# marcin-ochman/modular-slam

Hardware: AMD Instinct MI355X
Metric: ORB keypoints extracted+matched /sec, 640×480 RGB-D, 1/2/4/8 GPU; HBM GB/s vs roofline (higher is better)
Workload: dtype u8

## Files before the change

### modular-slam_amd/__init__.py

```python
import ctypes as C
import os
import subprocess

import numpy as np

_HERE = os.path.dirname(os.path.abspath(__file__))
LIB_PATH = os.path.join(_HERE, "libmslam_hip.so")

OK, E_INVALID, E_RUNTIME, E_CAPACITY, E_NO_VOCABULARY, E_FORMAT, E_NO_MODEL = range(7)
DBG_PYRAMID, DBG_BLURRED, DBG_CANDIDATES, DBG_SELECTED, DBG_CELLS, DBG_FORMS, DBG_QUAD_DIRECT = range(7)
QUAD_DIRECT_MAX_CANDIDATES = 1024
MATCHER_AUTO, MATCHER_POPCOUNT = 0, 1
DETECTOR_DISTRIBUTED, DETECTOR_CV_ORB = 0, 1
BOW_ASSIGN_TREE, BOW_ASSIGN_FLAT = 0, 1
CV_ORDER_LIBSTDCXX, CV_ORDER_RASTER = 0, 1
POSE_GRAPH_MAX_KEYFRAMES, POSE_GRAPH_MAX_EDGES = 1024, 65536

ABI_SYMBOLS = [
    "mslam_hip_default_params", "mslam_hip_abi_version", "mslam_hip_create", "mslam_hip_destroy",
    "mslam_hip_last_error", "mslam_hip_sync", "mslam_hip_detect", "mslam_hip_detect_batch_dev",
    "mslam_hip_get_batch_view", "mslam_hip_match", "mslam_hip_match_knn2", "mslam_hip_match_batch_dev",
    "mslam_hip_bow_load", "mslam_hip_bow_info", "mslam_hip_bow_words", "mslam_hip_bow_transform",
    "mslam_hip_bow_score", "mslam_hip_bow_db_add", "mslam_hip_bow_db_query", "mslam_hip_bow_db_clear",
    "mslam_hip_bow_batch_dev", "mslam_hip_get_bow_view", "mslam_hip_bow_cross_score_dev", "mslam_hip_level_geometry", "mslam_hip_debug_read",
    "mslam_hip_set_profiling", "mslam_hip_get_stage_times", "mslam_hip_copy_to_host", "mslam_hip_backproject", "mslam_hip_backproject_batch_dev",
    "mslam_hip_get_points_view", "mslam_hip_set_matcher", "mslam_hip_get_matcher",
    "mslam_hip_bow_pack_dev", "mslam_hip_bow_cross_score_packed_dev", "mslam_hip_debug_counts",
    "mslam_hip_last_match_kernel",
    "mslam_hip_join_matcher", "mslam_hip_bow_db_remove", "mslam_hip_bow_set_assignment",
    "mslam_hip_bow_db_reserve", "mslam_hip_bow_db_size", "mslam_hip_qlz_decompress",
    "mslam_hip_pnp_ransac", "mslam_hip_pnp_batch_dev", "mslam_hip_get_pnp_view", "mslam_hip_pnp_set_confidence", "mslam_hip_pack_batch_dev", "mslam_hip_packed_capacity",
    "mslam_hip_set_cv_keypoint_order", "mslam_hip_pnp_min_mse", "mslam_hip_pnp_min_mse_batch_dev",
    "mslam_hip_kf_add", "mslam_hip_kf_add_from_batch_dev", "mslam_hip_kf_remove", "mslam_hip_kf_clear", "mslam_hip_kf_size",
    "mslam_hip_kf_reserve", "mslam_hip_kf_read", "mslam_hip_relocalize",
    "mslam_hip_kf_visible", "mslam_hip_track", "mslam_hip_track_window", "mslam_hip_track_window_dev",
    "mslam_hip_kf_add_ids", "mslam_hip_kf_read_ids", "mslam_hip_kf_covisible", "mslam_hip_kf_union", "mslam_hip_kf_union_dev",
    "mslam_hip_match_guided_knn2", "mslam_hip_match_guided", "mslam_hip_set_guided_match", "mslam_hip_get_guided_match",
    "mslam_hip_bundle_adjust", "mslam_hip_bundle_adjust_global", "mslam_hip_kf_update_world", "mslam_hip_pose_graph",
]


class MslamHipError(RuntimeError):
    def __init__(self, code, msg):
        super().__init__("mslam_hip error %d: %s" % (code, msg))
        self.code = code


class Params(C.Structure):
    _fields_ = [("width", C.c_int32), ("height", C.c_int32), ("max_batch", C.c_int32), ("n_levels", C.c_int32),
                ("scale_factor", C.c_float), ("ini_fast_thr", C.c_int32), ("min_fast_thr", C.c_int32),
                ("min_node_area", C.c_uint32), ("max_keypoints", C.c_int32), ("max_candidates", C.c_int32),
                ("device", C.c_int32), ("stream", C.c_void_p), ("detector", C.c_int32), ("n_features", C.c_int32),
                ("edge_threshold", C.c_int32)]


class BatchView(C.Structure):
    _fields_ = [("n_frames", C.c_int32), ("capacity", C.c_int32), ("xy", C.c_void_p), ("desc", C.c_void_p),
                ("octave", C.c_void_p), ("angle", C.c_void_p), ("response", C.c_void_p), ("count", C.c_void_p),
                ("match_from", C.c_void_p), ("match_to", C.c_void_p), ("match_count", C.c_void_p)]


class PointsView(C.Structure):
    _fields_ = [("capacity", C.c_int32), ("xyz", C.c_void_p), ("valid", C.c_void_p)]

# ... 1298 lines not shown
```

### modular-slam_amd/csrc/api.hip

```cpp
#include "context.hpp"

#include <cfloat>
#include <climits>
#include <cmath>
#include <cstdio>
#include <cstring>
#include <cstdlib>
#include <algorithm>

using namespace mslam;

static thread_local std::string g_create_error;

#define ENTER(c)                                                                                                       \
    do                                                                                                                 \
    {                                                                                                                  \
        if(!(c))                                                                                                       \
            return MSLAM_HIP_E_INVALID;                                                                                \
        MSLAM_CHK(c, hipSetDevice((c)->p.device));                                                                     \
    } while(0)

static inline int cv_round_f(float v) { return (int)lrintf(v); }
static inline int cv_floor_f(float v)
{
// ... 616 lines not shown
        {
            const char* e = getenv("MSLAM_HIP_FUSED_LEVELS");
            const int want = e ? atoi(e) : kMaxLevels;
            const char* k = getenv("MSLAM_HIP_LEVEL_K6");
            const char* ks = getenv("MSLAM_HIP_LEVEL_K6_SMALL");
            c->level_k6_small = ks ? std::max(0, atoi(ks)) : 0;
            {
                const char* lc = getenv("MSLAM_HIP_LEVEL_CHAIN");
                const char* lf = getenv("MSLAM_HIP_LEVEL_CHAIN_FRAMES");
                const char* lw = getenv("MSLAM_HIP_LEVEL_CHAIN_WAVES");
                const char* lk = getenv("MSLAM_HIP_LEVEL_CHAIN_K6");
                c->level_chain = lc ? atoi(lc) : 0;
                c->level_chain_frames = lf ? std::max(1, std::min(64, atoi(lf))) : 2;
                c->level_chain_waves = lw ? atoi(lw) : 8;
                if(c->level_chain_waves != 4)
                    c->level_chain_waves = 8;
                c->level_chain_k6 = lk ? std::max(1, std::min(9, atoi(lk))) : 9;
            }
            c->level_k6 = k ? std::max(1, atoi(k)) : 5;
            const bool fits = (p.width & 3) == 0 && (double)B * p.width * p.height * 3 < 4294967296.0 &&
                              (double)B * g.slab < 4294901760.0  && (size_t)B * (p.width / 4) < (1u << 22) && p.height >= 8;
            int n_fused = fits ? 1 : 0;
            while(n_fused >= 1 && n_fused < p.n_levels && c->rs_q[n_fused] != SIZE_MAX && g.lv[n_fused].h >= 8 &&
                  (size_t)B * ((g.lv[n_fused].w + 3) / 4) < (1u << 22))
                ++n_fused;
            c->fused_levels = std::max(0, std::min(want, n_fused));
            const char* t = getenv("MSLAM_HIP_TILED_BLUR");
            c->geom.blur_tiled = c->fused_levels == p.n_levels && !(t && atoi(t) == 0) ? 1 : 0;
        }
        std::vector<BlurWave> bw;
        build_blur_waves(g, c->fused_levels, bw);
        c->blur_wpf = (int)bw.size();
        if(!bw.empty())
        {
            MSLAM_CHK(c, c->d_blur_waves.alloc(bw.size()));
            MSLAM_CHK(c, hipMemcpy(c->d_blur_waves, bw.data(), bw.size() * sizeof(BlurWave), hipMemcpyHostToDevice));
        }
    }
    MSLAM_CHK(c, c->d_cell_cnt.alloc(B * g.n_cells));
    MSLAM_CHK(c, c->d_cell_kp.alloc(B * g.n_cells * (size_t)kCellCap));
    QuadArgs& q = c->quad;
    MSLAM_CHK(c, c->q_cand.alloc(B * L * cap));
    MSLAM_CHK(c, c->q_cand_cnt.alloc(B * L));
    MSLAM_CHK(c, c->q_sel.alloc(B * L * cap));
    MSLAM_CHK(c, c->q_sel_cnt.alloc(B * L));
    MSLAM_CHK(c, c->q_kp_node.alloc(B * L * cap));
    MSLAM_CHK(c, c->q_nodes_a.alloc(B * L * cap));
    MSLAM_CHK(c, c->q_nodes_b.alloc(B * L * cap));
    MSLAM_CHK(c, c->q_ncnt_a.alloc(B * L * cap));
    MSLAM_CHK(c, c->q_ncnt_b.alloc(B * L * cap));
    MSLAM_CHK(c, c->q_child_cnt.alloc(B * L * cap * 4));
    MSLAM_CHK(c, c->q_ninfo.alloc(B * L * cap));
    MSLAM_CHK(c, c->q_best.alloc(B * L * cap));
    q.cand = c->q_cand, q.cand_cnt = c->q_cand_cnt, q.sel = c->q_sel, q.sel_cnt = c->q_sel_cnt, q.kp_node = c->q_kp_node;
    q.nodes_a = c->q_nodes_a, q.nodes_b = c->q_nodes_b, q.ncnt_a = c->q_ncnt_a, q.ncnt_b = c->q_ncnt_b;
    q.child_cnt = c->q_child_cnt, q.ninfo = c->q_ninfo, q.best = c->q_best;
    q.cell_cnt = c->d_cell_cnt;
    q.cell_kp = c->d_cell_kp;
    q.flags = c->d_flags;
    q.cand_cap = p.max_candidates;
    q.min_size = p.min_node_area;
    }

    for(auto& o : c->out)
    {
        MSLAM_CHK(c, o.xy.alloc((B + 1) * K * 2));
        MSLAM_CHK(c, o.desc.alloc((B + 1) * K * 32));
        MSLAM_CHK(c, o.octave.alloc((B + 1) * K));
        MSLAM_CHK(c, o.angle.alloc((B + 1) * K));
        MSLAM_CHK(c, o.response.alloc((B + 1) * K));
        MSLAM_CHK(c, o.count.alloc(B + 1));
        MSLAM_CHK(c, hipMemset(o.count, 0, (B + 1) * 4));
        MSLAM_CHK(c, o.idx0.alloc(B * K));
        MSLAM_CHK(c, o.idx1.alloc(B * K));
        MSLAM_CHK(c, o.dist0.alloc(B * K));
        MSLAM_CHK(c, o.dist1.alloc(B * K));
        MSLAM_CHK(c, o.mfrom.alloc(B * K));
        MSLAM_CHK(c, o.mto.alloc(B * K));
        MSLAM_CHK(c, o.mcount.alloc(B));
        MSLAM_CHK(c, hipMemset(o.mcount, 0, B * 4));
        MSLAM_CHK(c, hipEventCreateWithFlags(&o.ev_detect, hipEventDisableTiming));
        MSLAM_CHK(c, hipEventCreateWithFlags(&o.ev_match, hipEventDisableTiming));
    }
    MSLAM_CHK(c, hipStreamCreateWithFlags(&c->stream_m, hipStreamNonBlocking));
    {
        const char* e = getenv("MSLAM_HIP_OVERLAP_MATCH");
        c->overlap_match = !(e && atoi(e) == 0);
        auto on = [](const char* name) { const char* v = getenv(name); return !v || atoi(v) != 0; };
        c->knob_mirror_results = on("MSLAM_HIP_MIRROR_RESULTS");
        c->knob_zero_copy = on("MSLAM_HIP_ZERO_COPY_FRAME");
        c->knob_match_graph = on("MSLAM_HIP_MATCH_GRAPH");
        const char* zm = getenv("MSLAM_HIP_ZERO_COPY_MAX_BYTES");
        c->zero_copy_max_bytes = zm ? (size_t)atoll(zm) : (size_t)1200000;
        const char* m = getenv("MSLAM_HIP_MATCHER");
        c->matcher_kind = (m && std::strcmp(m, "popcount") == 0) ? MSLAM_HIP_MATCHER_POPCOUNT : MSLAM_HIP_MATCHER_AUTO;
    }
    c->cur = 0;
    MSLAM_CHK(c, hipDeviceSynchronize());
    return MSLAM_HIP_OK;
}

int mslam_hip_create(const mslam_hip_params* p, mslam_hip_ctx** out)
{
    if(!p || !out)
    {
        g_create_error = "null argument";
        return MSLAM_HIP_E_INVALID;
    }
    *out = nullptr;
// ... 1050 lines not shown
```

### modular-slam_amd/csrc/common.hpp

```cpp
#pragma once
#include <hip/hip_runtime.h>
#include <cstdint>
#include <cstddef>

namespace mslam
{

constexpr int kMaxLevels = 16;
constexpr int kBorder = 19;
constexpr int kCell = 64;
constexpr int kOverlap = 6;
constexpr int kCellCap = 1024;

constexpr size_t al256(size_t x) { return (x + 255) & ~(size_t)255; }

struct LevelGeom
{
    int w, h;
    int pitch;
    int offset;
    float scale;
    int bw, bh;
    int cell_base;
    int n_cells;
// ... 48 lines not shown
__host__ __device__ inline int kp_y(uint32_t p) { return (int)(p >> 20); }
__host__ __device__ inline int kp_score(uint32_t p) { return (int)(p & 0xFFu); }

enum : uint32_t
{
    kFlagCandOverflow = 1u,
    kFlagKpOverflow = 2u,
    kFlagQuadNoConverge = 4u,
    kFlagBowPackOverflow = 8u,
    kFlagDbFull = 16u,
    kFlagPackOverflow = 32u,
    kFlagUnionOverflow = 64u
};

void launch_gray(const uint8_t* d_bgr, uint8_t* d_pyr, const Geometry& g, int frame0, int n_frames, hipStream_t s);
void launch_resize(uint8_t* d_pyr, const Geometry& g, int level, const int32_t* d_xofs, const uint32_t* d_xcoef,
                   const int32_t* d_yofs, const uint32_t* d_ycoef, int frame0, int n_frames, hipStream_t s);
struct ResizeColArgs
{
    uint8_t* pyr;
    unsigned slab;
    int src_off, sh, spitch, dst_off, dw, dh, dpitch;
    const uint4* qt;
    const int32_t* yofs;
    const uint32_t* ycoef;
    int frame0, n_frames;
    int quads;
    float inv_quads;
    int R;
    int need_mask;
    int exact;
};
void launch_resize_col(const ResizeColArgs& a, hipStream_t s);
void launch_fast(const uint8_t* d_pyr, const Geometry& g, const CellDesc* d_cells, uint32_t* d_cell_cnt,
                 uint32_t* d_cell_kp, int ini_thr, int min_thr, int frame0, int n_frames, hipStream_t s);
void launch_denorm_selfcheck(uint32_t* d_out, hipStream_t s);
struct QuadArgs
{
    const uint32_t* cell_cnt;
    const uint32_t* cell_kp;
    uint32_t* cand;
    uint32_t* cand_cnt;
    uint32_t* sel;
    uint32_t* sel_cnt;
    uint32_t* kp_node;
    uint2* nodes_a;
    uint2* nodes_b;
    uint32_t* ncnt_a;
    uint32_t* ncnt_b;
    uint32_t* child_cnt;
    uint32_t* ninfo;
    uint32_t* best;
    uint32_t* flags;
    int cand_cap;
    unsigned min_size;
};
void launch_quadtree(const Geometry& g, const QuadArgs& a, int frame0, int n_frames, hipStream_t s);
int quad_depth_bound(const LevelGeom& lv, unsigned min_size);
unsigned quad_direct_levels(const Geometry& g);
struct BlurK
{
    uint32_t ta[3], tb[4], tc[4];
    uint32_t t01, t23, t45, t6;
};
BlurK make_blur_k();
struct GrayBlurArgs
{
    const uint8_t* bgr;
    uint8_t* pyr;
    uint8_t* blur;
    int W, H, pitch;
    unsigned slab;
    int n_frames, frame0;
    int quads;
    float inv_quads;
    int wide;
    int k6;
    int waves_per_xcd;
    int blur_tiled;
    BlurK bk;
};
void launch_gray_blur(const GrayBlurArgs& a, hipStream_t s);
struct ResizeBlurArgs
{
    uint8_t* pyr;
    uint8_t* blur;
    unsigned slab;
    int src_off, sh, spitch, dst_off, dw, dh, dpitch;
    const uint4* qt;
    const int32_t* yofs;
    const uint32_t* ycoef;
    int frame0, n_frames;
    int quads;
    float inv_quads;
    int wide;
    int k6;
    int need_mask;
    int exact;
    int waves_per_xcd;
    int blur_tiled;
    int always_load;
    BlurK bk;
};
void launch_resize_blur(const ResizeBlurArgs& a, hipStream_t s);
constexpr int kOctNeed = 0x48;
constexpr int kChainLevels = 8;
// ... 158 lines not shown
```

### modular-slam_amd/csrc/context.hpp

```cpp
#pragma once
#include "common.hpp"
#include "devmem.hpp"
#include "../../include/mslam_hip.h"
#include <array>
#include <string>
#include <vector>

namespace mslam
{
struct BowState;
void bow_destroy(BowState*);
struct RelocState;
void reloc_destroy(RelocState*);
void set_blur_taps(const int* taps);
void build_blur_waves(const Geometry& g, int first_level, std::vector<BlurWave>& out);

struct StageTimer
{
    const char* name;
    hipEvent_t start, stop;
};
}

struct mslam_out_set
// ... 13 lines not shown
{
    mslam_hip_params p{};
    mslam::Geometry geom{};
    hipStream_t stream = nullptr;
    bool own_stream = false;
    int n_side = 2;
    hipStream_t side[4] = {nullptr, nullptr, nullptr, nullptr};
    hipEvent_t ev_fork = nullptr, ev_join[4] = {nullptr, nullptr, nullptr, nullptr};
    hipStream_t blur_stream[4] = {nullptr, nullptr, nullptr, nullptr};
    hipEvent_t ev_blur_fork[4] = {nullptr, nullptr, nullptr, nullptr}, ev_blur_join[4] = {nullptr, nullptr, nullptr, nullptr};
    bool fork_blur = false;
    std::string err;

    std::vector<mslam::CellDesc> cells;

    mslam::DevBuf<mslam::CellDesc> d_cells;
    mslam::DevBuf<int32_t> d_rs_ofs;
    mslam::DevBuf<uint32_t> d_rs_coef;
    std::vector<size_t> rs_x, rs_y;
    mslam::DevBuf<uint4> d_rs_qt;
    std::vector<size_t> rs_q;
    std::vector<int> rs_need;
    mslam::DevBuf<uint4> d_rs_qt8;
    std::vector<size_t> rs_q8;
    mslam::DevBuf<int32_t> d_cv_ofs;
    mslam::DevBuf<uint32_t> d_cv_coef;
    std::vector<size_t> cv_x, cv_y;
    std::vector<std::array<int, 4>> cv_range;
    std::vector<int> cv_window12;
    int cv_quota[mslam::kMaxLevels] = {0};
    mslam::DevBuf<int32_t> d_ratio_thr;
    mslam::DevBuf<uint32_t> d_orient_w;
    hipGraphExec_t detect_graph[2] = {nullptr, nullptr};
    bool use_graph = true;
    int cv_order = 0;
    bool mirror_results = false;
    hipGraphExec_t match_graph = nullptr;
    int match_graph_from_cap = 0, match_graph_to_cap = 0, match_graph_kind = -1, match_graph_kernel = 0;
    mslam::PinnedBuf<uint8_t> h_out;
    double ratio_cached = -1.0;

    mslam::DevBuf<uint8_t> d_stage;
    mslam::PinnedBuf<uint8_t> h_stage;
    mslam::DevBuf<uint8_t> d_pyr, d_blur;
    mslam::DevBuf<mslam::BlurWave> d_blur_waves;
    int blur_wpf = 0;
    int fused_levels = 0;
    int level_k6 = 5;
    bool knob_mirror_results = true, knob_zero_copy = true, knob_match_graph = true;
    size_t zero_copy_max_bytes = 1200000;
    int level_chain = 0, level_chain_frames = 2, level_chain_waves = 8, level_chain_k6 = 9;
    int level_k6_small = 1;
    mslam::DevBuf<uint32_t> d_cell_cnt, d_cell_kp;
    mslam::DevBuf<uint32_t> q_cand, q_cand_cnt, q_sel, q_sel_cnt, q_kp_node, q_ncnt_a, q_ncnt_b, q_child_cnt, q_ninfo, q_best;
    mslam::DevBuf<uint2> q_nodes_a, q_nodes_b;
    mslam::QuadArgs quad{};
    mslam::DevBuf<uint32_t> d_flags;

    mslam_out_set out[2];
    int cur = 0;
    hipStream_t stream_m = nullptr;
    bool overlap_match = true;
    int matcher_kind = 0;
    int last_match_kernel = 0;
    double guided_radius = 0.0;
    int guided_max_distance = 256, guided_width = 0, guided_height = 0;
    int n_last = 0;
    unsigned long long detect_seq = 0;
    unsigned long long points_seq = ~0ull;
    unsigned long long match_seq = ~0ull;
    bool have_prev = false;

    mslam::DevBuf<uint8_t> d_hm_from;
    uint8_t* d_hm_to = nullptr;
    mslam::DevBuf<int32_t> d_hm_out;
    int hm_from_cap = 0, hm_to_cap = 0;
    mslam::DevBuf<uint32_t> d_hm_partial;
    mslam::PinnedBuf<uint8_t> h_hm;

    mslam::DevBuf<double> d_xyz;
    mslam::DevBuf<uint8_t> d_valid;
    mslam::DevBuf<float> d_pnp_obj, d_pnp_img;
    mslam::DevBuf<int32_t> d_pnp_n, d_pnp_counts;
    mslam::DevBuf<double> d_pnp_hyp, d_pnp_out;
    mslam::DevBuf<uint8_t> d_pnp_mask;
    int pnp_iterations = 0;
    double pnp_confidence = 0.99;
    mslam::DevBuf<float> d_pnp1_obj, d_pnp1_img;
    mslam::DevBuf<double> d_pnp1_hyp, d_pnp1_out;
    mslam::DevBuf<int32_t> d_pnp1_counts;
    mslam::DevBuf<uint8_t> d_pnp1_mask;
    int pnp1_n_cap = 0, pnp1_it_cap = 0;
    mslam::DevBuf<double> d_mse1;
    bool pnp_attr_set = false;
    mslam::DevBuf<uint8_t> d_ba;
    mslam::PinnedBuf<int32_t> h_ba;
    mslam::DevBuf<double> d_ba_S;
    mslam::DevBuf<uint8_t> d_pg;

    mslam::BowState* bow = nullptr;
    mslam::RelocState* reloc = nullptr;

    bool profiling = false;
    bool inplace_timing = false;
    std::vector<mslam::StageTimer> timers;
    size_t timers_used = 0;
};
// ... 78 lines not shown
```

### modular-slam_amd/csrc/k_quadtree.hip

```cpp
#include "common.hpp"
#include <algorithm>
#include <cstdlib>

namespace mslam
{

constexpr int QT = 512;
constexpr int kSmallKp = 512, kSmallQT = 256;
constexpr int kMidKp = 1024, kMidQT = 512;
constexpr int kLdsKp = 2048;
constexpr int kMaxCellsPerLevel = 2048;
constexpr int kBigNodes = 4096;
constexpr int kBigKp = 12288;
constexpr int kBigMinPixels = 400000;
constexpr int kMaxInitNodes = 64;
constexpr int kDirectKp = 1024, kDirectQT = 256, kDirectSlots = 1365, kDirectMaxDepth = 10;
constexpr int kMaxPasses = 40;

struct Scan
{
    uint32_t wsum[QT / 64];
};

__device__ __forceinline__ uint32_t wave_incl_scan(uint32_t v)
{
    int x = (int)v;
    x += __builtin_amdgcn_update_dpp(0, x, 0x111, 0xF, 0xF, true);
    x += __builtin_amdgcn_update_dpp(0, x, 0x112, 0xF, 0xF, true);
    x += __builtin_amdgcn_update_dpp(0, x, 0x114, 0xF, 0xE, true);
    x += __builtin_amdgcn_update_dpp(0, x, 0x118, 0xF, 0xC, true);
    x += __builtin_amdgcn_update_dpp(0, x, 0x142, 0xA, 0xF, true);
    x += __builtin_amdgcn_update_dpp(0, x, 0x143, 0xC, 0xF, true);
    return (uint32_t)x;
}

template <int NT>
__device__ __forceinline__ uint32_t block_excl_scan(uint32_t v, Scan& s, uint32_t& total)
{
    const int lane = threadIdx.x & 63, wave = threadIdx.x >> 6;
    const uint32_t inc = wave_incl_scan(v);
    if(lane == 63)
        s.wsum[wave] = inc;
    __syncthreads();
    uint32_t base = 0, tot = 0;
#pragma unroll
    for(int w = 0; w < NT / 64; ++w)
    {
        const uint32_t x = s.wsum[w];
        if(w < wave)
            base += x;
        tot += x;
    }
    __syncthreads();
    total = tot;
    return base + inc - v;
}

template <int NT>
__device__ __forceinline__ void block_excl_scan2(uint32_t a, uint32_t b, Scan& s, Scan& s2, uint32_t& exa, uint32_t& exb,
                                                 uint32_t& tota, uint32_t& totb)
{
    const int lane = threadIdx.x & 63, wave = threadIdx.x >> 6;
    const uint32_t ia = wave_incl_scan(a), ib = wave_incl_scan(b);
    if(lane == 63)
    {
        s.wsum[wave] = ia;
        s2.wsum[wave] = ib;
    }
    __syncthreads();
// ... 255 lines not shown
    if(!converged && n > 0 && tid == 0)
        atomicOr(a.flags, kFlagQuadNoConverge);

    for(uint32_t pos = tid; pos < n; pos += NT)
        best[pos] = 0;
    __syncthreads();
    for(uint32_t k = tid; k < N; k += NT)
    {
        const uint32_t pos = kp_node[k];
        if(pos == kNoNode)
            continue;
        atomicMax(&best[pos], ((uint32_t)kp_score(cand[k]) << 24) | (0xFFFFFFu - k));
    }
    __syncthreads();
    for(uint32_t pos = tid; pos < n; pos += NT)
    {
        const uint32_t k = 0xFFFFFFu - ((S::kLds ? best[pos] : ld_atomic(&best[pos])) & 0xFFFFFFu);
        sel[pos] = cand[k];
    }
    if(tid == 0)
        a.sel_cnt[slot] = n;
    return true;
}

template <int NT>
__device__ __forceinline__ uint32_t quad_cell_offsets(const uint32_t* ccnt, int n_cells, uint32_t* cell_off, Scan& scan)
{
    const int tid = threadIdx.x;
    uint32_t running = 0;
    for(int base = 0; base < n_cells; base += NT)
    {
        const int i = base + tid;
        const uint32_t v = i < n_cells ? ccnt[i] : 0u;
        uint32_t tot;
        const uint32_t ex = block_excl_scan<NT>(v, scan, tot);
        if(i < n_cells)
            cell_off[i] = running + ex;
        running += tot;
    }
    if(tid == 0)
        cell_off[n_cells] = running;
    __syncthreads();
    return running;
}

__device__ __forceinline__ int quad_class(uint32_t N, int n_cells, unsigned classes)
{
    if((classes & 1u) && N <= (uint32_t)kSmallKp && n_cells <= 2 * kSmallKp - 1)
        return 0;
    if((classes & 2u) && N <= (uint32_t)kMidKp && n_cells <= 2 * kMidKp - 1)
        return 1;
    return 2;
}
template <int KP, int NT, int CLS>
__global__ __launch_bounds__(NT) __attribute__((amdgpu_waves_per_eu(CLS == 2 ? 4 : 8))) void k_quadtree(Geometry g, QuadArgs a, unsigned big_levels, unsigned direct_levels)
{
    __shared__ Scan scan, scan2;
    __shared__ uint32_t l_cand[KP];
    __shared__ uint2 l_nodes_a[KP], l_nodes_b[KP];
    __shared__ uint32_t l_cc[KP * 2];
    __shared__ uint16_t l_kp_node[KP], l_ncnt_a[KP], l_ncnt_b[KP], l_nbase[KP];
    __shared__ uint8_t l_ninfo[KP];
    __shared__ uint32_t init_cnt[kMaxInitNodes];
    __shared__ uint32_t init_pos[kMaxInitNodes];
    __shared__ uint32_t sh_n;
    constexpr int kCellsFit = 2 * KP - 1;
    static_assert(CLS != 2 || kCellsFit >= kMaxCellsPerLevel, "cell offsets must fit");
    const unsigned classes = big_levels >> 30;
    uint32_t* cell_off = reinterpret_cast<uint32_t*>(l_nodes_b);

    const int level = (int)((blockIdx.x + blockIdx.y) % (unsigned)g.n_levels);
    const size_t frame = blockIdx.y + g.frame0;
    const LevelGeom& lv = g.lv[level];
    const int tid = threadIdx.x;
    const size_t slot = frame * g.n_levels + level;
    const size_t cap = (size_t)a.cand_cap;
    uint32_t* cand = a.cand + slot * cap;
    uint32_t* sel = a.sel + slot * cap;

    const int n_cells = lv.n_cells;
    if(n_cells > kCellsFit)
        return;
    const uint32_t* ccnt = a.cell_cnt + frame * g.n_cells + lv.cell_base;
    const uint32_t N = quad_cell_offsets<NT>(ccnt, n_cells, cell_off, scan);
    if(((direct_levels >> level) & 1u) && N <= (uint32_t)kDirectKp)
        return;
    if(quad_class(N, n_cells, classes) != CLS)
        return;
    if(N > (uint32_t)a.cand_cap)
    {
        if(tid == 0)
        {
            atomicOr(a.flags, kFlagCandOverflow);
            a.cand_cnt[slot] = 0;
            a.sel_cnt[slot] = 0;
        }
        return;
    }
    if(tid == 0)
        a.cand_cnt[slot] = N;
    if(N == 0)
    {
        if(tid == 0)
            a.sel_cnt[slot] = 0;
        return;
    }
    if(N <= (uint32_t)KP)
        quad_run<LdsStore, NT>(g, a, lv, frame, slot, tid, N, n_cells, cell_off, l_cand, cand, l_kp_node, l_nodes_a, l_nodes_b,
                               l_ncnt_a, l_ncnt_b, l_ninfo, l_nbase, l_cc, l_cc, sel, scan, scan2, init_cnt, init_pos, sh_n);
    else if((big_levels >> level) & 1u)
        return;
    else
        quad_run<GlobalStore, NT>(g, a, lv, frame, slot, tid, N, n_cells, cell_off, cand, cand, a.kp_node + slot * cap,
                                  a.nodes_a + slot * cap, a.nodes_b + slot * cap, a.ncnt_a + slot * cap,
                                  a.ncnt_b + slot * cap, a.ninfo + slot * cap, a.best + slot * cap,
                                  a.child_cnt + slot * cap * 4, a.best + slot * cap, sel, scan, scan2, init_cnt, init_pos,
                                  sh_n);
}

__global__ __launch_bounds__(QT) void k_quadtree_big(Geometry g, QuadArgs a, unsigned big_levels)
{
    extern __shared__ __attribute__((aligned(16))) uint8_t big_lds[];
    __shared__ Scan scan, scan2;
    __shared__ uint32_t init_cnt[kMaxInitNodes];
    __shared__ uint32_t init_pos[kMaxInitNodes];
    __shared__ uint32_t sh_n;
    uint2* l_nodes_a = reinterpret_cast<uint2*>(big_lds);
    uint2* l_nodes_b = l_nodes_a + kBigNodes;
    uint32_t* l_cc = reinterpret_cast<uint32_t*>(l_nodes_b + kBigNodes);
    uint16_t* l_kp_node = reinterpret_cast<uint16_t*>(l_cc + 2 * kBigNodes);
    uint16_t* l_ncnt_a = l_kp_node + kBigKp;
    uint16_t* l_ncnt_b = l_ncnt_a + kBigNodes;
    uint16_t* l_nbase = l_ncnt_b + kBigNodes;
    uint8_t* l_ninfo = reinterpret_cast<uint8_t*>(l_nbase + kBigNodes);
    static_assert(kBigNodes * sizeof(uint2) >= (kMaxCellsPerLevel + 1) * sizeof(uint32_t), "cell offsets must fit");
    uint32_t* cell_off = reinterpret_cast<uint32_t*>(l_nodes_b);

    int level = 0;
    {
        unsigned m = big_levels;
        const unsigned which = (blockIdx.x + blockIdx.y) % gridDim.x;
        for(unsigned i = 0; i < which; ++i)
            m &= m - 1;
        level = __ffs((int)m) - 1;
    }
    const size_t frame = blockIdx.y + g.frame0;
    const LevelGeom& lv = g.lv[level];
    const int tid = threadIdx.x;
    const size_t slot = frame * g.n_levels + level;
    const size_t cap = (size_t)a.cand_cap;
    uint32_t* cand = a.cand + slot * cap;
    uint32_t* sel = a.sel + slot * cap;
    const int n_cells = lv.n_cells;
    const uint32_t* ccnt = a.cell_cnt + frame * g.n_cells + lv.cell_base;
    const uint32_t N = quad_cell_offsets<QT>(ccnt, n_cells, cell_off, scan);
    if(N <= (uint32_t)kLdsKp || N > (uint32_t)a.cand_cap)
        return;
    bool done = false;
    if(N <= (uint32_t)kBigKp)
        done = quad_run<BigStore, QT>(g, a, lv, frame, slot, tid, N, n_cells, cell_off, cand, cand, l_kp_node, l_nodes_a, l_nodes_b,
                                  l_ncnt_a, l_ncnt_b, l_ninfo, l_nbase, l_cc, l_cc, sel, scan, scan2, init_cnt, init_pos, sh_n);
    if(!done)
    {
        __syncthreads();
        quad_cell_offsets<QT>(ccnt, n_cells, cell_off, scan);
        quad_run<GlobalStore, QT>(g, a, lv, frame, slot, tid, N, n_cells, cell_off, cand, cand, a.kp_node + slot * cap,
                              a.nodes_a + slot * cap, a.nodes_b + slot * cap, a.ncnt_a + slot * cap,
                              a.ncnt_b + slot * cap, a.ninfo + slot * cap, a.best + slot * cap,
                              a.child_cnt + slot * cap * 4, a.best + slot * cap, sel, scan, scan2, init_cnt, init_pos,
                              sh_n);
    }
}

template <int SLOTS>
struct DirectTable
{
    uint32_t cnt[(SLOTS + 1) / 2];
    uint32_t best[SLOTS];
    uint8_t flag[SLOTS];
};

__device__ __forceinline__ uint32_t direct_block_start(uint32_t n_init, int d) { return n_init * (((1u << (2 * d)) - 1u) / 3u); }

template <int KP, int SLOTS, int NT>
__global__ __launch_bounds__(NT) __attribute__((amdgpu_waves_per_eu(8))) void k_quadtree_direct(Geometry g, QuadArgs a, unsigned direct_levels)
{
    constexpr int PER = KP / NT;
    static_assert(KP % NT == 0 && KP == kDirectKp, "instance shape");
    __shared__ Scan scan;
    __shared__ uint32_t l_cand[KP];
    __shared__ DirectTable<SLOTS> t;
    __shared__ uint32_t tot[2 * (kDirectMaxDepth + 2)];

    const int level = (int)((blockIdx.x + blockIdx.y) % (unsigned)g.n_levels);
    if(!((direct_levels >> level) & 1u))
        return;
    const size_t frame = blockIdx.y + g.frame0;
    const LevelGeom& lv = g.lv[level];
    const int tid = threadIdx.x;
    const size_t slot = frame * g.n_levels + level;
    const size_t cap = (size_t)a.cand_cap;
    uint32_t* g_cand = a.cand + slot * cap;
    uint32_t* sel = a.sel + slot * cap;
    const int D = lv.qdepth;
    const uint32_t n_init = (uint32_t)(lv.nxg * lv.nyg);
    const uint32_t n_slots = direct_block_start(n_init, D + 1);

    for(uint32_t i = tid; i < (n_slots + 1) / 2; i += NT)
        t.cnt[i] = 0;
    for(uint32_t i = tid; i < n_slots; i += NT)
        t.flag[i] = 0;
    if(tid < 2 * (kDirectMaxDepth + 2))
        tot[tid] = 0;

    const int n_cells = lv.n_cells;
    uint32_t* cell_off = t.best;
    const uint32_t* ccnt = a.cell_cnt + frame * g.n_cells + lv.cell_base;
    const uint32_t N = quad_cell_offsets<NT>(ccnt, n_cells, cell_off, scan);
    if(N > (uint32_t)KP)
        return;
    if(N > (uint32_t)a.cand_cap)
    {
        if(tid == 0)
        {
            atomicOr(a.flags, kFlagCandOverflow);
            a.cand_cnt[slot] = 0;
            a.sel_cnt[slot] = 0;
        }
        return;
    }
    if(tid == 0)
        a.cand_cnt[slot] = N;
    if(N == 0)
    {
        if(tid == 0)
            a.sel_cnt[slot] = 0;
        return;
    }

    const uint32_t* ckp = a.cell_kp + (frame * g.n_cells + lv.cell_base) * (size_t)kCellCap;
    const float sf = lv.scale;
    const float min_size_f = (float)a.min_size;
    uint32_t path[PER];
#pragma unroll
    for(int i = 0; i < PER; ++i)
    {
        const uint32_t k = (uint32_t)(tid + i * NT);
        path[i] = ~0u;
        if(k >= N)
            continue;
        int lo = 0, hi = n_cells - 1;
        while(lo < hi)
        {
            const int mid = (lo + hi + 1) >> 1;
            if(cell_off[mid] <= k)
                lo = mid;
            else
                hi = mid - 1;
        }
        const uint32_t p = ckp[(size_t)lo * kCellCap + (k - cell_off[lo])];
        l_cand[k] = p;
        g_cand[k] = p;
        const int x = kp_x(p), y = kp_y(p);
        const unsigned ix = (unsigned)((double)(float)x / lv.delta_x);
        const unsigned iy = (unsigned)((double)(float)y / lv.delta_y);
        const unsigned idx = ix + iy * (unsigned)lv.nxg;
        if(idx >= n_init)
            continue;
        int bx = (int)(lv.delta_x * ix), by = (int)(lv.delta_y * iy);
        int ex = (int)(lv.delta_x * (ix + 1)), ey = (int)(lv.delta_y * (iy + 1));
        uint32_t q = idx;
        int d = 0;
        for(;;)
        {
            const uint32_t s = direct_block_start(n_init, d) + q;
            atomicAdd(&t.cnt[s >> 1], 1u << (16 * (s & 1u)));
            const unsigned area = (unsigned)((ex - bx) * (ey - by));
            if(__fmul_rn(__fmul_rn((float)area, sf), sf) <= min_size_f || d == D)
            {
                t.flag[s] = 1;
                break;
            }
            const int cx = bx + ((ex - bx + 1) >> 1), cy = by + ((ey - by + 1) >> 1);
            const bool right = cx <= x, low = cy <= y;
            bx = right ? cx : bx, ex = right ? ex : cx;
            by = low ? cy : by, ey = low ? ey : cy;
            q = (q << 2) | (right ? 1u : 0u) | (low ? 2u : 0u);
            ++d;
        }
        path[i] = ((uint32_t)d << 24) | q;
    }
    __syncthreads();

    for(int d = 0; d <= D; ++d)
    {
        const uint32_t start = direct_block_start(n_init, d), n_d = n_init << (2 * d);
        const uint32_t pstart = direct_block_start(n_init, d > 0 ? d - 1 : 0);
        uint32_t kd = 0, md = 0;
        for(uint32_t base = 0; base < n_d; base += NT)
        {
            const uint32_t q = base + tid;
            bool keep = false, open = false;
            if(q < n_d)
            {
                const uint32_t s = start + q, ps = pstart + (q >> 2);
                const uint32_t c = (t.cnt[s >> 1] >> (16 * (s & 1u))) & 0xFFFFu;
                const uint32_t pc = d > 0 ? (t.cnt[ps >> 1] >> (16 * (ps & 1u))) & 0xFFFFu : 2u;
                const bool real = c > 0 && pc >= 2;
                keep = real && (c == 1 || t.flag[s] != 0);
                open = real && !keep;
                t.flag[s] = keep ? 1 : open ? 2 : 0;
                t.best[s] = 0;
            }
            kd += (uint32_t)__popcll(__ballot(keep));
            md += (uint32_t)__popcll(__ballot(open));
        }
        if((tid & 63) == 0 && (kd | md) != 0)
        {
            atomicAdd(&tot[2 * d], kd);
            atomicAdd(&tot[2 * d + 1], md);
        }
    }
    __syncthreads();
    int P = 1;
    while(tot[2 * P] + tot[2 * P + 1] != tot[2 * P - 1])
        ++P;
    const int top = P < D ? P : D;

#pragma unroll
    for(int i = 0; i < PER; ++i)
    {
        if(path[i] == ~0u)
            continue;
        const uint32_t k = (uint32_t)(tid + i * NT);
        const int dk = (int)(path[i] >> 24);
        const uint32_t q = path[i] & 0xFFFFFFu;
        const int last = dk < top ? dk : top;
        uint32_t leaf = 0;
        for(int d = 0; d <= last; ++d)
        {
            leaf = direct_block_start(n_init, d) + (q >> (2 * (dk - d)));
            if(t.flag[leaf] == 1)
                break;
        }
        atomicMax(&t.best[leaf], ((uint32_t)kp_score(l_cand[k]) << 24) | (0xFFFFFFu - k));
    }
    __syncthreads();

    const uint32_t n_entries = direct_block_start(n_init, top + 1);
    const uint32_t per = (n_entries + NT - 1) / NT;
    const uint32_t e0 = (uint32_t)tid * per, e1 = e0 + per < n_entries ? e0 + per : n_entries;
    auto entry_slot = [&](uint32_t e, bool& is_leaf) {
        int d = top;
        uint32_t n_d = n_init << (2 * d);
        while(e >= n_d)
        {
            e -= n_d;
            --d;
            n_d >>= 2;
        }
        const uint32_t bits = 2u * (uint32_t)d, low_mask = (1u << bits) - 1u;
        uint32_t i0 = e >> bits;
        if(d & 1)
            i0 = n_init - 1u - i0;
        const uint32_t s = direct_block_start(n_init, d) + ((i0 << bits) | ((e ^ 0x33333333u) & low_mask));
        const uint32_t f = t.flag[s];
        is_leaf = f == 1 || (f == 2 && d == P);
        return s;
    };
    uint32_t mine = 0;
    for(uint32_t e = e0; e < e1; ++e)
    {
        bool is_leaf;
        entry_slot(e, is_leaf);
        mine += is_leaf ? 1u : 0u;
    }
    uint32_t n_leaves;
    uint32_t r = block_excl_scan<NT>(mine, scan, n_leaves);
    for(uint32_t e = e0; e < e1 && mine != 0; ++e)
    {
        bool is_leaf;
        const uint32_t s = entry_slot(e, is_leaf);
        if(is_leaf)
            sel[r++] = l_cand[0xFFFFFFu - (t.best[s] & 0xFFFFFFu)];
    }
    if(tid == 0)
        a.sel_cnt[slot] = n_leaves;
}

unsigned quad_direct_levels(const Geometry& g)
{
    const char* env = getenv("MSLAM_HIP_QUAD_DIRECT");
    const bool on = !env || atoi(env) != 0;
    unsigned m = 0;
    for(int l = 0; on && l < g.n_levels; ++l)
    {
        const LevelGeom& lv = g.lv[l];
        if(lv.qdepth < 0 || lv.qdepth > kDirectMaxDepth || lv.n_cells + 1 > kDirectSlots)
            continue;
        const long long slots = (long long)lv.nxg * lv.nyg * (((1ll << (2 * (lv.qdepth + 1))) - 1) / 3);
        if(slots <= kDirectSlots)
            m |= 1u << l;
    }
    return m;
}

int quad_depth_bound(const LevelGeom& lv, unsigned min_size)
{
    int dx = 0, dy = 0;
    for(int iy = 0; iy < lv.nyg; ++iy)
        for(int ix = 0; ix < lv.nxg; ++ix)
        {
            dx = std::max(dx, (int)(lv.delta_x * (ix + 1)) - (int)(lv.delta_x * ix));
            dy = std::max(dy, (int)(lv.delta_y * (iy + 1)) - (int)(lv.delta_y * iy));
        }
    for(int d = 0; d <= 15; ++d)
    {
        const unsigned area = (unsigned)(dx * dy);
        const float scaled = (float)area * lv.scale;
        if(scaled * lv.scale <= (float)min_size)
            return d;
        if(dx <= 1 && dy <= 1)
            break;
        dx = (dx + 1) >> 1, dy = (dy + 1) >> 1;
    }
    return -1;
}

void launch_quadtree(const Geometry& g, const QuadArgs& a, int frame0, int n_frames, hipStream_t s)
{
    dim3 grid(g.n_levels, n_frames);
    Geometry gg = g;
    gg.frame0 = frame0;
    unsigned big_levels = 0;
    for(int l = 0; l < g.n_levels; ++l)
        if(g.lv[l].w * g.lv[l].h > kBigMinPixels)
            big_levels |= 1u << l;
    static const unsigned classes_env = [] { const char* e = getenv("MSLAM_HIP_QUAD_CLASSES"); return e ? (unsigned)atoi(e) & 3u : 3u; }();
    const unsigned direct = quad_direct_levels(g);
    const bool all_direct = direct == (g.n_levels >= 32 ? ~0u : (1u << g.n_levels) - 1u);
    const unsigned classes = n_frames < 8 || all_direct ? 0u : classes_env;
    const unsigned bl = big_levels | (classes << 30);
    if(direct != 0)
        hipLaunchKernelGGL((k_quadtree_direct<kDirectKp, kDirectSlots, kDirectQT>), grid, dim3(kDirectQT), 0, s, gg, a, direct);
    hipLaunchKernelGGL((k_quadtree<kLdsKp, QT, 2>), grid, dim3(QT), 0, s, gg, a, bl, direct);
    if(classes & 2u)
        hipLaunchKernelGGL((k_quadtree<kMidKp, kMidQT, 1>), grid, dim3(kMidQT), 0, s, gg, a, bl, direct);
    if(classes & 1u)
        hipLaunchKernelGGL((k_quadtree<kSmallKp, kSmallQT, 0>), grid, dim3(kSmallQT), 0, s, gg, a, bl, direct);
    if(big_levels != 0)
    {
        constexpr size_t lds = (size_t)kBigNodes * (8 + 8 + 8 + 2 + 2 + 2 + 1) + (size_t)kBigKp * 2;
        static const bool attr = [] {
            return hipFuncSetAttribute((const void*)k_quadtree_big, hipFuncAttributeMaxDynamicSharedMemorySize, (int)lds) == hipSuccess;
        }();
        (void)attr;
        hipLaunchKernelGGL(k_quadtree_big, dim3((unsigned)__builtin_popcount(big_levels), n_frames), dim3(QT), lds, s, gg, a,
                           big_levels);
    }
}

}
```

Baseline: 666.1 million.

## Route oversized direct quadtree pairs through a compact todo-list kernel

The direct quadtree kernel's capacity doubles, and it handles small inputs with half its per-thread slots active. Level/frame pairs that exceed its capacity are now appended to a device-side todo list instead of being rescanned by full-grid fallback kernels. A persistent kernel sized to about two workgroups per CU drains that list, and the full-grid LDS quadtree launches are skipped when every level is direct. This cuts empty workgroup launches and redundant cell-offset scans, at the cost of more LDS in the direct kernel and an atomic counter reset protocol.

```diff
diff --git a/modular-slam_amd/__init__.py b/modular-slam_amd/__init__.py
--- a/modular-slam_amd/__init__.py
+++ b/modular-slam_amd/__init__.py
@@ -10,6 +10,7 @@
 OK, E_INVALID, E_RUNTIME, E_CAPACITY, E_NO_VOCABULARY, E_FORMAT, E_NO_MODEL = range(7)
 DBG_PYRAMID, DBG_BLURRED, DBG_CANDIDATES, DBG_SELECTED, DBG_CELLS, DBG_FORMS, DBG_QUAD_DIRECT = range(7)
 QUAD_DIRECT_MAX_CANDIDATES = 1024
+QUAD_DIRECT_CAPACITY = 2048
 MATCHER_AUTO, MATCHER_POPCOUNT = 0, 1
 DETECTOR_DISTRIBUTED, DETECTOR_CV_ORB = 0, 1
 BOW_ASSIGN_TREE, BOW_ASSIGN_FLAT = 0, 1
diff --git a/modular-slam_amd/csrc/api.hip b/modular-slam_amd/csrc/api.hip
--- a/modular-slam_amd/csrc/api.hip
+++ b/modular-slam_amd/csrc/api.hip
@@ -692,9 +692,11 @@
     MSLAM_CHK(c, c->q_child_cnt.alloc(B * L * cap * 4));
     MSLAM_CHK(c, c->q_ninfo.alloc(B * L * cap));
     MSLAM_CHK(c, c->q_best.alloc(B * L * cap));
+    MSLAM_CHK(c, c->q_todo.alloc(B * (L + 2)));
+    MSLAM_CHK(c, hipMemset(c->q_todo, 0, B * (L + 2) * sizeof(uint32_t)));
     q.cand = c->q_cand, q.cand_cnt = c->q_cand_cnt, q.sel = c->q_sel, q.sel_cnt = c->q_sel_cnt, q.kp_node = c->q_kp_node;
     q.nodes_a = c->q_nodes_a, q.nodes_b = c->q_nodes_b, q.ncnt_a = c->q_ncnt_a, q.ncnt_b = c->q_ncnt_b;
-    q.child_cnt = c->q_child_cnt, q.ninfo = c->q_ninfo, q.best = c->q_best;
+    q.child_cnt = c->q_child_cnt, q.ninfo = c->q_ninfo, q.best = c->q_best, q.todo = c->q_todo;
     q.cell_cnt = c->d_cell_cnt;
     q.cell_kp = c->d_cell_kp;
     q.flags = c->d_flags;
diff --git a/modular-slam_amd/csrc/common.hpp b/modular-slam_amd/csrc/common.hpp
--- a/modular-slam_amd/csrc/common.hpp
+++ b/modular-slam_amd/csrc/common.hpp
@@ -124,6 +124,7 @@
     uint32_t* ninfo;
     uint32_t* best;
     uint32_t* flags;
+    uint32_t* todo;
     int cand_cap;
     unsigned min_size;
 };
diff --git a/modular-slam_amd/csrc/context.hpp b/modular-slam_amd/csrc/context.hpp
--- a/modular-slam_amd/csrc/context.hpp
+++ b/modular-slam_amd/csrc/context.hpp
@@ -89,7 +89,7 @@
     int level_chain = 0, level_chain_frames = 2, level_chain_waves = 8, level_chain_k6 = 9;
     int level_k6_small = 1;
     mslam::DevBuf<uint32_t> d_cell_cnt, d_cell_kp;
-    mslam::DevBuf<uint32_t> q_cand, q_cand_cnt, q_sel, q_sel_cnt, q_kp_node, q_ncnt_a, q_ncnt_b, q_child_cnt, q_ninfo, q_best;
+    mslam::DevBuf<uint32_t> q_cand, q_cand_cnt, q_sel, q_sel_cnt, q_kp_node, q_ncnt_a, q_ncnt_b, q_child_cnt, q_ninfo, q_best, q_todo;
     mslam::DevBuf<uint2> q_nodes_a, q_nodes_b;
     mslam::QuadArgs quad{};
     mslam::DevBuf<uint32_t> d_flags;
diff --git a/modular-slam_amd/csrc/k_quadtree.hip b/modular-slam_amd/csrc/k_quadtree.hip
--- a/modular-slam_amd/csrc/k_quadtree.hip
+++ b/modular-slam_amd/csrc/k_quadtree.hip
@@ -14,7 +14,7 @@
 constexpr int kBigKp = 12288;
 constexpr int kBigMinPixels = 400000;
 constexpr int kMaxInitNodes = 64;
-constexpr int kDirectKp = 1024, kDirectQT = 256, kDirectSlots = 1365, kDirectMaxDepth = 10;
+constexpr int kDirectKp = 2048, kDirectQT = 256, kDirectSlots = 1365, kDirectMaxDepth = 10;
 constexpr int kMaxPasses = 40;
 
 struct Scan
@@ -376,41 +376,44 @@
         return 1;
     return 2;
 }
-template <int KP, int NT, int CLS>
-__global__ __launch_bounds__(NT) __attribute__((amdgpu_waves_per_eu(CLS == 2 ? 4 : 8))) void k_quadtree(Geometry g, QuadArgs a, unsigned big_levels, unsigned direct_levels)
-{
-    __shared__ Scan scan, scan2;
-    __shared__ uint32_t l_cand[KP];
-    __shared__ uint2 l_nodes_a[KP], l_nodes_b[KP];
-    __shared__ uint32_t l_cc[KP * 2];
-    __shared__ uint16_t l_kp_node[KP], l_ncnt_a[KP], l_ncnt_b[KP], l_nbase[KP];
-    __shared__ uint8_t l_ninfo[KP];
-    __shared__ uint32_t init_cnt[kMaxInitNodes];
-    __shared__ uint32_t init_pos[kMaxInitNodes];
-    __shared__ uint32_t sh_n;
-    constexpr int kCellsFit = 2 * KP - 1;
-    static_assert(CLS != 2 || kCellsFit >= kMaxCellsPerLevel, "cell offsets must fit");
-    const unsigned classes = big_levels >> 30;
-    uint32_t* cell_off = reinterpret_cast<uint32_t*>(l_nodes_b);
-
-    const int level = (int)((blockIdx.x + blockIdx.y) % (unsigned)g.n_levels);
-    const size_t frame = blockIdx.y + g.frame0;
+template <int KP>
+struct QuadLds
+{
+    Scan scan, scan2;
+    uint32_t cand[KP];
+    uint2 nodes_a[KP], nodes_b[KP];
+    uint32_t cc[KP * 2];
+    uint16_t kp_node[KP], ncnt_a[KP], ncnt_b[KP], nbase[KP];
+    uint8_t ninfo[KP];
+    uint32_t init_cnt[kMaxInitNodes];
+    uint32_t init_pos[kMaxInitNodes];
+    uint32_t sh_n;
+    static constexpr int kCellsFit = 2 * KP - 1;
+    __device__ __forceinline__ uint32_t* cell_off() { return reinterpret_cast<uint32_t*>(nodes_b); }
+};
+
+template <>
+struct QuadLds<0>
+{
+    Scan scan, scan2;
+    uint32_t off[kMaxCellsPerLevel + 1];
+    uint32_t init_cnt[kMaxInitNodes];
+    uint32_t init_pos[kMaxInitNodes];
+    uint32_t sh_n;
+    static constexpr int kCellsFit = kMaxCellsPerLevel;
+    __device__ __forceinline__ uint32_t* cell_off() { return off; }
+};
+
+template <int KP, int NT>
+__device__ __forceinline__ void quad_pair(const Geometry& g, const QuadArgs& a, QuadLds<KP>& l, int level, size_t frame,
+                                          uint32_t N, unsigned big_levels)
+{
     const LevelGeom& lv = g.lv[level];
     const int tid = threadIdx.x;
     const size_t slot = frame * g.n_levels + level;
     const size_t cap = (size_t)a.cand_cap;
     uint32_t* cand = a.cand + slot * cap;
     uint32_t* sel = a.sel + slot * cap;
-
-    const int n_cells = lv.n_cells;
-    if(n_cells > kCellsFit)
-        return;
-    const uint32_t* ccnt = a.cell_cnt + frame * g.n_cells + lv.cell_base;
-    const uint32_t N = quad_cell_offsets<NT>(ccnt, n_cells, cell_off, scan);
-    if(((direct_levels >> level) & 1u) && N <= (uint32_t)kDirectKp)
-        return;
-    if(quad_class(N, n_cells, classes) != CLS)
-        return;
     if(N > (uint32_t)a.cand_cap)
     {
         if(tid == 0)
@@ -429,17 +432,75 @@
             a.sel_cnt[slot] = 0;
         return;
     }
-    if(N <= (uint32_t)KP)
-        quad_run<LdsStore, NT>(g, a, lv, frame, slot, tid, N, n_cells, cell_off, l_cand, cand, l_kp_node, l_nodes_a, l_nodes_b,
-                               l_ncnt_a, l_ncnt_b, l_ninfo, l_nbase, l_cc, l_cc, sel, scan, scan2, init_cnt, init_pos, sh_n);
-    else if((big_levels >> level) & 1u)
+    if constexpr(KP > 0)
+    {
+        if(N <= (uint32_t)KP)
+        {
+            quad_run<LdsStore, NT>(g, a, lv, frame, slot, tid, N, lv.n_cells, l.cell_off(), l.cand, cand, l.kp_node, l.nodes_a,
+                                   l.nodes_b, l.ncnt_a, l.ncnt_b, l.ninfo, l.nbase, l.cc, l.cc, sel, l.scan, l.scan2,
+                                   l.init_cnt, l.init_pos, l.sh_n);
+            return;
+        }
+    }
+    if((big_levels >> level) & 1u)
         return;
     else
-        quad_run<GlobalStore, NT>(g, a, lv, frame, slot, tid, N, n_cells, cell_off, cand, cand, a.kp_node + slot * cap,
+        quad_run<GlobalStore, NT>(g, a, lv, frame, slot, tid, N, lv.n_cells, l.cell_off(), cand, cand, a.kp_node + slot * cap,
                                   a.nodes_a + slot * cap, a.nodes_b + slot * cap, a.ncnt_a + slot * cap,
                                   a.ncnt_b + slot * cap, a.ninfo + slot * cap, a.best + slot * cap,
-                                  a.child_cnt + slot * cap * 4, a.best + slot * cap, sel, scan, scan2, init_cnt, init_pos,
-                                  sh_n);
+                                  a.child_cnt + slot * cap * 4, a.best + slot * cap, sel, l.scan, l.scan2, l.init_cnt,
+                                  l.init_pos, l.sh_n);
+}
+
+template <int KP, int NT, int CLS>
+__global__ __launch_bounds__(NT) __attribute__((amdgpu_waves_per_eu(CLS == 2 ? 4 : 8))) void k_quadtree(Geometry g, QuadArgs a, unsigned big_levels, unsigned direct_levels)
+{
+    __shared__ QuadLds<KP> l;
+    static_assert(CLS != 2 || QuadLds<KP>::kCellsFit >= kMaxCellsPerLevel, "cell offsets must fit");
+    const unsigned classes = big_levels >> 30;
+
+    const int level = (int)((blockIdx.x + blockIdx.y) % (unsigned)g.n_levels);
+    if((direct_levels >> level) & 1u)
+        return;
+    const size_t frame = blockIdx.y + g.frame0;
+    const LevelGeom& lv = g.lv[level];
+
+    const int n_cells = lv.n_cells;
+    if(n_cells > QuadLds<KP>::kCellsFit)
+        return;
+    const uint32_t* ccnt = a.cell_cnt + frame * g.n_cells + lv.cell_base;
+    const uint32_t N = quad_cell_offsets<NT>(ccnt, n_cells, l.cell_off(), l.scan);
+    if(quad_class(N, n_cells, classes) != CLS)
+        return;
+    quad_pair<KP, NT>(g, a, l, level, frame, N, big_levels);
+}
+
+template <int KP, int NT>
+__global__ __launch_bounds__(NT) void k_quadtree_todo(Geometry g, QuadArgs a, unsigned big_levels)
+{
+    __shared__ QuadLds<KP> l;
+    static_assert(QuadLds<KP>::kCellsFit >= kMaxCellsPerLevel, "cell offsets must fit");
+    static_assert(KP >= kLdsKp || (KP == 0 && kDirectKp >= kLdsKp), "a listed pair that fits the LDS arrays must find them");
+    uint32_t* list = a.todo + (size_t)g.frame0 * (size_t)(g.n_levels + 2);
+    const uint32_t n = (uint32_t)__builtin_amdgcn_readfirstlane((int)ld_atomic(&list[0]));
+    if(n == 0)
+        return;
+    for(uint32_t e = blockIdx.x; e < n; e += gridDim.x)
+    {
+        const uint32_t pair = (uint32_t)__builtin_amdgcn_readfirstlane((int)list[2 + e]);
+        const int level = (int)(pair % (uint32_t)g.n_levels);
+        const size_t frame = pair / (uint32_t)g.n_levels;
+        const LevelGeom& lv = g.lv[level];
+        const uint32_t* ccnt = a.cell_cnt + frame * g.n_cells + lv.cell_base;
+        const uint32_t N = quad_cell_offsets<NT>(ccnt, lv.n_cells, l.cell_off(), l.scan);
+        quad_pair<KP, NT>(g, a, l, level, frame, N, big_levels);
+        __syncthreads();
+    }
+    if(threadIdx.x == 0 && atomicAdd(&list[1], 1u) == gridDim.x - 1u)
+    {
+        atomicExch(&list[1], 0u);
+        atomicExch(&list[0], 0u);
+    }
 }
 
 __global__ __launch_bounds__(QT) void k_quadtree_big(Geometry g, QuadArgs a, unsigned big_levels)
@@ -510,7 +571,7 @@
 __global__ __launch_bounds__(NT) __attribute__((amdgpu_waves_per_eu(8))) void k_quadtree_direct(Geometry g, QuadArgs a, unsigned direct_levels)
 {
     constexpr int PER = KP / NT;
-    static_assert(KP % NT == 0 && KP == kDirectKp, "instance shape");
+    static_assert(KP % (2 * NT) == 0 && KP == kDirectKp, "instance shape");
     __shared__ Scan scan;
     __shared__ uint32_t l_cand[KP];
     __shared__ DirectTable<SLOTS> t;
@@ -541,8 +602,6 @@
     uint32_t* cell_off = t.best;
     const uint32_t* ccnt = a.cell_cnt + frame * g.n_cells + lv.cell_base;
     const uint32_t N = quad_cell_offsets<NT>(ccnt, n_cells, cell_off, scan);
-    if(N > (uint32_t)KP)
-        return;
     if(N > (uint32_t)a.cand_cap)
     {
         if(tid == 0)
@@ -561,6 +620,16 @@
             a.sel_cnt[slot] = 0;
         return;
     }
+    if(N > (uint32_t)KP)
+    {
+        if(tid == 0)
+        {
+            uint32_t* list = a.todo + (size_t)g.frame0 * (size_t)(g.n_levels + 2);
+            list[2 + atomicAdd(&list[0], 1u)] = (uint32_t)slot;
+        }
+        return;
+    }
+    const bool wide = __builtin_amdgcn_readfirstlane((int)N) > KP / 2;
 
     const uint32_t* ckp = a.cell_kp + (frame * g.n_cells + lv.cell_base) * (size_t)kCellCap;
     const float sf = lv.scale;
@@ -571,6 +640,8 @@
     {
         const uint32_t k = (uint32_t)(tid + i * NT);
         path[i] = ~0u;
+        if(i >= PER / 2 && !wide)
+            continue;
         if(k >= N)
             continue;
         int lo = 0, hi = n_cells - 1;
@@ -654,6 +725,8 @@
 #pragma unroll
     for(int i = 0; i < PER; ++i)
     {
+        if(i >= PER / 2 && !wide)
+            break;
         if(path[i] == ~0u)
             continue;
         const uint32_t k = (uint32_t)(tid + i * NT);
@@ -751,6 +824,17 @@
     return -1;
 }
 
+static int quad_cu_count()
+{
+    static int cus[64] = {0};
+    int dev = 0, n = 0;
+    if(hipGetDevice(&dev) != hipSuccess || dev < 0 || dev >= 64)
+        return 256;
+    if(cus[dev] == 0)
+        cus[dev] = hipDeviceGetAttribute(&n, hipDeviceAttributeMultiprocessorCount, dev) == hipSuccess && n > 0 ? n : 256;
+    return cus[dev];
+}
+
 void launch_quadtree(const Geometry& g, const QuadArgs& a, int frame0, int n_frames, hipStream_t s)
 {
     dim3 grid(g.n_levels, n_frames);
@@ -763,15 +847,24 @@
     static const unsigned classes_env = [] { const char* e = getenv("MSLAM_HIP_QUAD_CLASSES"); return e ? (unsigned)atoi(e) & 3u : 3u; }();
     const unsigned direct = quad_direct_levels(g);
     const bool all_direct = direct == (g.n_levels >= 32 ? ~0u : (1u << g.n_levels) - 1u);
-    const unsigned classes = n_frames < 8 || all_direct ? 0u : classes_env;
+    const unsigned classes = n_frames < 8 ? 0u : classes_env;
     const unsigned bl = big_levels | (classes << 30);
     if(direct != 0)
+    {
         hipLaunchKernelGGL((k_quadtree_direct<kDirectKp, kDirectSlots, kDirectQT>), grid, dim3(kDirectQT), 0, s, gg, a, direct);
-    hipLaunchKernelGGL((k_quadtree<kLdsKp, QT, 2>), grid, dim3(QT), 0, s, gg, a, bl, direct);
-    if(classes & 2u)
-        hipLaunchKernelGGL((k_quadtree<kMidKp, kMidQT, 1>), grid, dim3(kMidQT), 0, s, gg, a, bl, direct);
-    if(classes & 1u)
-        hipLaunchKernelGGL((k_quadtree<kSmallKp, kSmallQT, 0>), grid, dim3(kSmallQT), 0, s, gg, a, bl, direct);
+        int wgs = std::min(g.n_levels * n_frames, 2 * quad_cu_count());
+        if(const char* e = getenv("MSLAM_HIP_QUAD_TODO_WGS"))
+            wgs = std::max(1, std::min(wgs, atoi(e)));
+        hipLaunchKernelGGL((k_quadtree_todo<kDirectKp >= kLdsKp ? 0 : kLdsKp, QT>), dim3((unsigned)wgs), dim3(QT), 0, s, gg, a, big_levels);
+    }
+    if(!all_direct)
+    {
+        hipLaunchKernelGGL((k_quadtree<kLdsKp, QT, 2>), grid, dim3(QT), 0, s, gg, a, bl, direct);
+        if(classes & 2u)
+            hipLaunchKernelGGL((k_quadtree<kMidKp, kMidQT, 1>), grid, dim3(kMidQT), 0, s, gg, a, bl, direct);
+        if(classes & 1u)
+            hipLaunchKernelGGL((k_quadtree<kSmallKp, kSmallQT, 0>), grid, dim3(kSmallQT), 0, s, gg, a, bl, direct);
+    }
     if(big_levels != 0)
     {
         constexpr size_t lds = (size_t)kBigNodes * (8 + 8 + 8 + 2 + 2 + 2 + 1) + (size_t)kBigKp * 2;
```

New measurement: 669.6 million (median of 6 runs). About the same (+0.5%).
